# thunguyenphuoc/RenderNet

Hardware: AMD Instinct MI355X
Metric: rendered frames/sec, 64^3 voxel->512x512 Phong, batch 24 (higher is better)
Workload: dtype f32 (multiply stages: bf16x3-split operands, fp32 accumulate); 1 GPU; Phong shader forward (resampler + RenderNet 1-ch head), 5 shipped binvox fixtures cycled, 64^3 -> 128^3 -> 512x512, seeded random weights (237.3M params); batch_per_gpu=24, global_batch=24

## Files before the change

rendernet_amd/csrc/conv3d_wino_bf3.hip:

```cpp
#include "wino_xform.h"
#include <stdlib.h>
#include <type_traits>

typedef _Float16 f16x2 __attribute__((ext_vector_type(2)));

namespace {
constexpr int C3 = 32;
constexpr int C3PW = 34, C3PH = 4;
constexpr int C3NPIX = C3PW * C3PH;
constexpr int C3NPIECE = 17;
constexpr int C3STAGE = 18 * 1024;
constexpr int C3NSTG = 3;
constexpr int C3XCH = 4 * 2 * 2 * 2 * 1024;
constexpr int C3TAB = 256;
constexpr unsigned C3OOB = 0x80000000u;
}

struct C3Args {
    const float* x; const char* u; const float* bias; const float* alpha; const float* res; float* y; float* z;
    unsigned x_bytes;
    int B, H, W, D;
    int bh, bw;
    int nitems;
    int nseg, seglen;
    int act;
    const unsigned* amax_x; const unsigned* amax_u;
    unsigned* amax_y;
};

struct C3B3 : rnf::FmtB3 {};
struct C3H2 : rnf::FmtH2 {};
constexpr float C3_BOUND_X = 4.f, C3_BOUND_U = 2.25f;

__host__ __device__ inline float c3_h2_scale(float amax, float bound)
{
    const float t = amax * bound * (1.0f / 32768.0f);
    if (!(t > 0.f)) return 1.f;
    int e;
    const float m = frexpf(t, &e);
    return ldexpf(1.f, m == 0.5f ? e - 1 : e);
}

__global__ __launch_bounds__(256)
void conv3d_wino_pack_bf3_kernel(const float* __restrict__ w_tf, unsigned short* __restrict__ us, int transposed)
{
    const int idx = blockIdx.x * blockDim.x + threadIdx.x;
    if (idx >= 16 * 3 * C3 * C3) return;
    const int n = idx % C3, c = (idx / C3) % C3, dz = (idx / (C3 * C3)) % 3, xi = idx / (C3 * C3 * 3);
    const int i = xi >> 2, j = xi & 3;
    const double G[4][3] = {{1.0, 0.0, 0.0}, {0.5, 0.5, 0.5}, {0.5, -0.5, 0.5}, {0.0, 0.0, 1.0}};
    double acc = 0.0;
    for (int p = 0; p < 3; ++p)
        for (int q = 0; q < 3; ++q) {
            const float w = transposed ? w_tf[((((size_t)(2 - p) * 3 + (2 - q)) * 3 + (2 - dz)) * C3 + n) * C3 + c]
                                       : w_tf[((((size_t)p * 3 + q) * 3 + dz) * C3 + c) * C3 + n];
            acc = __builtin_fma(G[i][p] * G[j][q], (double)w, acc);
        }
    const float u = (float)acc;
    const __bf16 h0 = (__bf16)u;
    const float r1 = u - (float)h0;
    const __bf16 h1 = (__bf16)r1;
    const float r2 = r1 - (float)h1;
    const __bf16 h2 = (__bf16)r2;
    const __bf16 h[3] = {h0, h1, h2};
    const int lane = (n & 15) + 16 * (c >> 3), nt = n >> 4, e = c & 7;
    for (int p = 0; p < 3; ++p)
        us[((((((size_t)i * 4 + j) * 3 + dz) * 3 + p) * 2 + nt) * 64 + lane) * 8 + e] = __builtin_bit_cast(unsigned short, h[p]);
}

__global__ __launch_bounds__(256)
void conv3d_wino_pack_h2_kernel(const float* __restrict__ w_tf, unsigned short* __restrict__ us, const unsigned* __restrict__ amax, int transposed)
{
    const int idx = blockIdx.x * blockDim.x + threadIdx.x;
    if (idx >= 16 * 3 * C3 * C3) return;
    const float inv = 1.f / c3_h2_scale(__builtin_bit_cast(float, *amax), C3_BOUND_U);
    const int n = idx % C3, c = (idx / C3) % C3, dz = (idx / (C3 * C3)) % 3, xi = idx / (C3 * C3 * 3);
    const int i = xi >> 2, j = xi & 3;
    const double G[4][3] = {{1.0, 0.0, 0.0}, {0.5, 0.5, 0.5}, {0.5, -0.5, 0.5}, {0.0, 0.0, 1.0}};
    double acc = 0.0;
    for (int p = 0; p < 3; ++p)
        for (int q = 0; q < 3; ++q) {
            const float w = transposed ? w_tf[((((size_t)(2 - p) * 3 + (2 - q)) * 3 + (2 - dz)) * C3 + n) * C3 + c]
                                       : w_tf[((((size_t)p * 3 + q) * 3 + dz) * C3 + c) * C3 + n];
            acc = __builtin_fma(G[i][p] * G[j][q], (double)w, acc);
        }
    const float u = (float)acc * inv;
    const _Float16 h0 = (_Float16)u;
    const _Float16 h1 = (_Float16)(u - (float)h0);
    const _Float16 h[2] = {h0, h1};
    const int lane = (n & 15) + 16 * (c >> 3), nt = n >> 4, e = c & 7;
    for (int p = 0; p < 2; ++p)
        us[((((((size_t)i * 4 + j) * 3 + dz) * 2 + p) * 2 + nt) * 64 + lane) * 8 + e] = __builtin_bit_cast(unsigned short, h[p]);
}

__device__ __forceinline__ void c3_split8(const f32x4 lo, const f32x4 hi, bf16x8 (&p)[3])
{
#pragma unroll
    for (int e = 0; e < 8; e += 2) {
        f32x2 v = e < 4 ? f32x2{lo[e], lo[e + 1]} : f32x2{hi[e - 4], hi[e - 3]};
        const bf16x2 h0 = __builtin_convertvector(v, bf16x2);
        v -= __builtin_convertvector(h0, f32x2);
        const bf16x2 h1 = __builtin_convertvector(v, bf16x2);
        v -= __builtin_convertvector(h1, f32x2);
        const bf16x2 h2 = __builtin_convertvector(v, bf16x2);
        p[0][e] = h0[0]; p[0][e + 1] = h0[1];
        p[1][e] = h1[0]; p[1][e + 1] = h1[1];
        p[2][e] = h2[0]; p[2][e + 1] = h2[1];
    }
}

__device__ __forceinline__ void c3_split8(const f32x4 lo, const f32x4 hi, float inv, f16x8 (&p)[2])
{
#pragma unroll
    for (int e = 0; e < 8; e += 2) {
        f32x2 v = (e < 4 ? f32x2{lo[e], lo[e + 1]} : f32x2{hi[e - 4], hi[e - 3]}) * inv;
        const f16x2 h0 = __builtin_convertvector(v, f16x2);
        v -= __builtin_convertvector(h0, f32x2);
        const f16x2 h1 = __builtin_convertvector(v, f16x2);
        p[0][e] = h0[0]; p[0][e + 1] = h0[1];
        p[1][e] = h1[0]; p[1][e + 1] = h1[1];
    }
}
__device__ __forceinline__ void c3_split8(const f32x4 lo, const f32x4 hi, float, bf16x8 (&p)[3]) { c3_split8(lo, hi, p); }

__device__ __forceinline__ void c3_mfma(f32x4& c, const bf16x8& u, const bf16x8& p)
{
    asm("s_nop 1\n\tv_mfma_f32_16x16x32_bf16 %0, %1, %2, %0" : "+v"(c) : "a"(u), "v"(p));
}
__device__ __forceinline__ void c3_mfma_start(f32x4& c, const bf16x8& u, const bf16x8& p)
{
    asm("s_nop 1\n\tv_mfma_f32_16x16x32_bf16 %0, %1, %2, 0" : "=v"(c) : "v"(u), "v"(p));
}
__device__ __forceinline__ void c3_mfma(f32x4& c, const f16x8& u, const f16x8& p)
{
    asm("s_nop 1\n\tv_mfma_f32_16x16x32_f16 %0, %1, %2, %0" : "+v"(c) : "a"(u), "v"(p));
}
__device__ __forceinline__ void c3_mfma_start(f32x4& c, const f16x8& u, const f16x8& p)
{
    asm("s_nop 1\n\tv_mfma_f32_16x16x32_f16 %0, %1, %2, 0" : "=v"(c) : "a"(u), "v"(p));
}

__device__ __forceinline__ int c3_slot_swap(int px) { return ((px >> 4) | (px >> 5)) & 1; }

#define C3_WAIT_BARRIER(N) asm volatile("s_waitcnt vmcnt(" #N ") lgkmcnt(0)\n\ts_barrier" ::: "memory")

template <class F, bool AMAX>
__global__ __launch_bounds__(512, 1)
void conv3d_wino_bf3_kernel(const C3Args a)
{
    typedef typename F::frag frag;
    constexpr int NP = F::NP;
#if defined(__HIP_DEVICE_COMPILE__)
    extern __shared__ __attribute__((aligned(16))) char smem[];
    typedef __attribute__((address_space(3))) void lds_void;
    typedef unsigned u32x4 __attribute__((ext_vector_type(4)));
    const int tid = threadIdx.x;
    const int lane = tid & 63, wave = __builtin_amdgcn_readfirstlane(tid >> 6);
    const int r = wave >> 1, c = wave & 1;
    const int tx = lane & 15, kq = lane >> 4;
    const __amdgpu_buffer_rsrc_t xrsrc = __builtin_amdgcn_make_buffer_rsrc(const_cast<float*>(a.x), 0, a.x_bytes, 0x00020000);
    const __amdgpu_buffer_rsrc_t yrsrc = __builtin_amdgcn_make_buffer_rsrc(a.y, 0, a.x_bytes, 0x00020000);
    const __amdgpu_buffer_rsrc_t zrsrc = __builtin_amdgcn_make_buffer_rsrc(a.z ? a.z : a.y, 0, a.x_bytes, 0x00020000);
    const __amdgpu_buffer_rsrc_t rrsrc = __builtin_amdgcn_make_buffer_rsrc(const_cast<float*>(a.res ? a.res : a.x), 0, a.x_bytes, 0x00020000);

    frag U[2][3][NP][2];
    {
        const frag* up = reinterpret_cast<const frag*>(a.u) + (size_t)(r * 4 + 2 * c) * (3 * NP * 2 * 64) + lane;
#pragma unroll
        for (int jj = 0; jj < 2; ++jj)
#pragma unroll
            for (int dz = 0; dz < 3; ++dz)
#pragma unroll
                for (int p = 0; p < NP; ++p)
#pragma unroll
                    for (int nt = 0; nt < 2; ++nt) U[jj][dz][p][nt] = up[(((jj * 3 + dz) * NP + p) * 2 + nt) * 64];
    }
    float inv_x = 1.f, out_scale = 1.f;
    if constexpr (F::ID == 1) {
        const float sx = c3_h2_scale(__builtin_bit_cast(float, *a.amax_x), C3_BOUND_X);
        inv_x = 1.f / sx;
        out_scale = sx * c3_h2_scale(__builtin_bit_cast(float, *a.amax_u), C3_BOUND_U);
    }
    float ymax = 0.f;
    float* tab = reinterpret_cast<float*>(smem + C3NSTG * C3STAGE + 2 * C3XCH);
    if (tid < C3) {
        tab[tid] = a.bias ? a.bias[tid] : 0.f;
        tab[C3 + tid] = a.alpha ? a.alpha[tid] : 0.f;
    }
    const int rowA = (0x1210 >> (4 * r)) & 3, rowB = (0x3122 >> (4 * r)) & 3;
    const float sgn = r == 1 ? 1.f : -1.f;
    unsigned fo[3][2];
#pragma unroll
    for (int k = 0; k < 3; ++k)
#pragma unroll
        for (int h = 0; h < 2; ++h) {
            const int b = c + k;
            const int px = 2 * tx + b;
            fo[k][h] = (unsigned)((px ^ c3_slot_swap(px)) * 128) + ((((unsigned)(2 * kq + h)) ^ (unsigned)((px >> 1) & 7)) << 4);
        }
    const unsigned offA = (unsigned)(rowA * C3PW * 128), offB = (unsigned)(rowB * C3PW * 128);

    const int G = gridDim.x;
    const unsigned pix_bytes = (unsigned)a.D * (C3 * 4);
    const bool three = wave == 0;
    const int ent = wave >> 2, dy = (wave >> 1) & 1, dx = wave & 1;
    const int nch = ent * 16 + 4 * kq;
    __syncthreads();

    f32x4 acc[3][2][2];
    const int perm = (int)(blockIdx.x & 7) * (G >> 3) + (int)(blockIdx.x >> 3);
    for (int id = perm; id < a.nitems; id += G) {
        const int bx = id % a.bw, by = (id / a.bw) % a.bh, bi = (id / (a.bw * a.bh)) % a.B, seg = id / (a.bw * a.bh * a.B);
        const int o0 = seg * a.seglen, o1 = o0 + a.seglen < a.D ? o0 + a.seglen : a.D;
        if (o0 >= o1) continue;
        const int ds = o0 > 0 ? o0 - 1 : 0, dl = o1 < a.D ? o1 : a.D - 1;
        const int y0 = by * 2 - 1, x0 = bx * 32 - 1;
        const unsigned base = (unsigned)((bi * a.H + y0) * a.W + x0) * pix_bytes;
        unsigned roff[3];
#pragma unroll
        for (int i = 0; i < 3; ++i) {
            const int q = (wave + 8 * i) * 8 + (lane >> 3);
            const int py = (q * 241) >> 13, pxs = q - py * C3PW;
            const int px = pxs ^ c3_slot_swap(pxs);
            const bool ok = q < C3NPIX && (unsigned)(y0 + py) < (unsigned)a.H && (unsigned)(x0 + px) < (unsigned)a.W;
            roff[i] = ok ? base + (unsigned)(py * a.W + px) * pix_bytes + (unsigned)((((lane & 7) ^ ((px >> 1) & 7))) << 4) : C3OOB;
        }
        const int oy = by * 2 + dy, ox = bx * 32 + 2 * tx + dx;
        const unsigned ooff = (oy < a.H && ox < a.W) ? (unsigned)((bi * a.H + oy) * a.W + ox) * pix_bytes + (unsigned)(nch * 4) : C3OOB;

        auto issue = [&](int d, int stage) {
            char* sb = smem + stage * C3STAGE;
#pragma unroll
            for (int i = 0; i < 3; ++i) {
                if (i == 2 && !three) break;
                __builtin_amdgcn_raw_ptr_buffer_load_lds(xrsrc, (lds_void*)(sb + (wave + 8 * i) * 1024), 16,
                                                         roff[i] + (unsigned)(d * (C3 * 4)), 0, 0, 0);
            }
        };
        auto wait_newest = [&](bool issued) {
            if (!issued) C3_WAIT_BARRIER(0);
            else if (three) C3_WAIT_BARRIER(3);
            else C3_WAIT_BARRIER(2);
        };
        issue(ds, 0);
        if (ds + 1 <= dl) issue(ds + 1, 1);
#pragma unroll
        for (int jj = 0; jj < 2; ++jj)
#pragma unroll
            for (int nt = 0; nt < 2; ++nt) acc[0][jj][nt] = f32x4{0.f, 0.f, 0.f, 0.f};
        wait_newest(ds + 1 <= dl);

        auto step = [&](auto sc, int d) {
            constexpr int S = decltype(sc)::value;
            constexpr int SP = (S + 2) % 3, SN = (S + 1) % 3;
            const bool fl = d > o0;
            const bool arith = d <= dl;
            f32x4 rv = {0.f, 0.f, 0.f, 0.f};
            if (fl && a.res) rv = __builtin_bit_cast(f32x4, __builtin_amdgcn_raw_buffer_load_b128(rrsrc, ooff, (d - 1) * (C3 * 4), 0));
            asm volatile("" ::: "memory");
            const bool issued = d + 2 <= dl;
            if (issued) issue(d + 2, SP);
            if (arith) {
                const char* sb = smem + S * C3STAGE;
                f32x4 v[2][2];
#pragma unroll
                for (int h = 0; h < 2; ++h) {
                    f32x4 t[3];
#pragma unroll
                    for (int k = 0; k < 3; ++k) {
                        const f32x4 dA = *reinterpret_cast<const f32x4*>(sb + fo[k][h] + offA);
                        const f32x4 dB = *reinterpret_cast<const f32x4*>(sb + fo[k][h] + offB);
                        t[k] = dA + sgn * dB;
                    }
                    if (c == 0) { v[0][h] = t[0] - t[2]; v[1][h] = t[1] + t[2]; }
                    else        { v[0][h] = t[1] - t[0]; v[1][h] = t[0] - t[2]; }
                }
#pragma unroll
                for (int jj = 0; jj < 2; ++jj) {
                    frag p[NP];
                    c3_split8(v[jj][0], v[jj][1], inv_x, p);
#pragma unroll
                    for (int k = 0; k < F::NPROD; ++k)
#pragma unroll
                        for (int nt = 0; nt < 2; ++nt) {
                            c3_mfma(acc[SP][jj][nt], U[jj][2][F::PU[k]][nt], p[F::PV[k]]);
                            c3_mfma(acc[S][jj][nt], U[jj][1][F::PU[k]][nt], p[F::PV[k]]);
                            if (k == 0) c3_mfma_start(acc[SN][jj][nt], U[jj][0][F::PU[k]][nt], p[F::PV[k]]);
                            else c3_mfma(acc[SN][jj][nt], U[jj][0][F::PU[k]][nt], p[F::PV[k]]);
                        }
                }
            }
            char* xch = smem + C3NSTG * C3STAGE + (d & 1) * C3XCH;
            if (fl) {
                asm volatile("s_nop 15\n\ts_nop 15" : "+v"(acc[SP][0][0]), "+v"(acc[SP][0][1]), "+v"(acc[SP][1][0]), "+v"(acc[SP][1][1]) :: "memory");
#pragma unroll
                for (int nt = 0; nt < 2; ++nt) {
                    const f32x4 m0 = acc[SP][0][nt], m1 = acc[SP][1][nt], s = m0 + m1;
                    const f32x4 p0 = c == 0 ? s : m0, p1 = c == 0 ? m1 : -s;
                    *reinterpret_cast<f32x4*>(xch + ((((r * 2 + 0) * 2 + c) * 2 + nt) * 64 + lane) * 16) = p0;
                    *reinterpret_cast<f32x4*>(xch + ((((r * 2 + 1) * 2 + c) * 2 + nt) * 64 + lane) * 16) = p1;
                }
            }
            wait_newest(issued);
            if (fl) {
                f32x4 ci[3];
#pragma unroll
                for (int k = 0; k < 3; ++k)
                    ci[k] = *reinterpret_cast<const f32x4*>(xch + (((((dy + k) * 2 + dx) * 2 + 0) * 2 + ent) * 64 + lane) * 16)
                          + *reinterpret_cast<const f32x4*>(xch + (((((dy + k) * 2 + dx) * 2 + 1) * 2 + ent) * 64 + lane) * 16);
                f32x4 o = (dy == 0 ? (ci[0] + ci[1]) + ci[2] : (ci[0] - ci[1]) - ci[2]);
                if constexpr (F::ID == 1) o *= out_scale;
                o += *reinterpret_cast<const f32x4*>(tab + nch);
                const unsigned so = ooff + (unsigned)((d - 1) * (C3 * 4));
                if (a.z) __builtin_amdgcn_raw_buffer_store_b128(__builtin_bit_cast(u32x4, o), zrsrc, so, 0, 0);
                if (a.act & RN_ACT_PRELU) {
                    const f32x4 av = *reinterpret_cast<const f32x4*>(tab + C3 + nch);
#pragma unroll
                    for (int e = 0; e < 4; ++e) o[e] = fmaxf(o[e], 0.f) + av[e] * fminf(o[e], 0.f);
                }
                if (a.act & RN_ACT_ELU) {
#pragma unroll
                    for (int e = 0; e < 4; ++e) o[e] = o[e] > 0.f ? o[e] : expf(o[e]) - 1.f;
                }
                if (a.res) o += rv;
                if (a.act & RN_ACT_SIGMOID) {
#pragma unroll
                    for (int e = 0; e < 4; ++e) o[e] = 1.f / (1.f + __expf(-o[e]));
                }
                __builtin_amdgcn_raw_buffer_store_b128(__builtin_bit_cast(u32x4, o), yrsrc, so, 0, 0);
                if (AMAX && ooff != C3OOB) ymax = fmaxf(fmaxf(ymax, fmaxf(fabsf(o[0]), fabsf(o[1]))), fmaxf(fabsf(o[2]), fabsf(o[3])));
            }
        };
        for (int d = ds; d <= o1; d += 3) {
            step(std::integral_constant<int, 0>{}, d);
            if (d + 1 <= o1) step(std::integral_constant<int, 1>{}, d + 1);
            if (d + 2 <= o1) step(std::integral_constant<int, 2>{}, d + 2);
        }
    }
    if (AMAX) {
#pragma unroll
        for (int o = 32; o > 0; o >>= 1) ymax = fmaxf(ymax, __shfl_xor(ymax, o));
        if (lane == 0) atomicMax(a.amax_y, __builtin_bit_cast(unsigned, ymax));
    }
#endif
}

bool rn_conv3d_wino_bf3_supported(int Cin, int Cout)
{
    return Cin == C3 && Cout == C3;
}

size_t rn_conv3d_wino_bf3_packed_bytes() { return (size_t)16 * 3 * C3 * C3 * 3 * 2; }
size_t rn_conv3d_wino_split_packed_bytes(int fmt) { return fmt == 1 ? (size_t)16 * 3 * C3 * C3 * 2 * 2 + 256 : rn_conv3d_wino_bf3_packed_bytes(); }

int rn_launch_conv3d_wino_pack_bf3(const float* w_tf, void* us, int transposed, hipStream_t st)
{
    return rn_launch_conv3d_wino_split_pack(0, w_tf, us, transposed, st);
}

int rn_launch_conv3d_wino_split_pack(int fmt, const float* w_tf, void* us, int transposed, hipStream_t st)
{
    if (fmt == 1) {
        unsigned* amax = reinterpret_cast<unsigned*>(static_cast<char*>(us) + (size_t)16 * 3 * C3 * C3 * 2 * 2);
        const int rc = rn_launch_absmax(w_tf, (size_t)27 * C3 * C3, amax, st);
        if (rc != RN_OK) return rc;
        hipLaunchKernelGGL(conv3d_wino_pack_h2_kernel, dim3((16 * 3 * C3 * C3 + 255) / 256), dim3(256), 0, st, w_tf,
                           static_cast<unsigned short*>(us), amax, transposed);
        return rn_check_launch("conv3d_wino_pack_h2");
    }
    hipLaunchKernelGGL(conv3d_wino_pack_bf3_kernel, dim3((16 * 3 * C3 * C3 + 255) / 256), dim3(256), 0, st, w_tf,
                       static_cast<unsigned short*>(us), transposed);
    return rn_check_launch("conv3d_wino_pack_bf3");
}

int rn_launch_conv3d_wino_bf3(const float* x, const void* us, const float* bias, const float* alpha, const float* residual,
                              float* y, float* preact, int B, int H, int W, int D, int act, hipStream_t st)
{
    return rn_launch_conv3d_wino_split(0, x, us, bias, alpha, residual, y, preact, B, H, W, D, act, nullptr, nullptr, nullptr, st);
}

static int c3_depth_segments(long long rows, int D)
{
    static const int forced = getenv("RN_C3_DEPTH_SEGMENTS") ? atoi(getenv("RN_C3_DEPTH_SEGMENTS")) : 0;
    if (forced >= 1) return forced < D ? forced : D;
    int best = 1;
    long long best_cost = 0;
    for (int n = 1; n <= 8 && n <= D; n *= 2) {
        const int len = (D + n - 1) / n;
        const long long rounds = (rows * n + 255) / 256;
        const long long cost = rounds * (len + (n > 1 ? 2 : 1) + 1);
        if (n == 1 || cost < best_cost) { best = n; best_cost = cost; }
    }
    return best;
}

int rn_launch_conv3d_wino_split(int fmt, const float* x, const void* us, const float* bias, const float* alpha, const float* residual,
                                float* y, float* preact, int B, int H, int W, int D, int act, const unsigned* amax_x, unsigned* scratch_amax,
                                unsigned* amax_y, hipStream_t st)
{
    if (B < 1 || H < 1 || W < 1 || D < 1) return rn_set_error(RN_E_INVALID, "conv3d_wino_bf3: bad sizes");
    if ((act & RN_ACT_PRELU) && !alpha) return rn_set_error(RN_E_INVALID, "conv3d_wino_bf3: PReLU needs alpha");
    if (fmt < 0 || fmt > 1) return rn_set_error(RN_E_INVALID, "conv3d_wino_bf3: operand format %d", fmt);
    const size_t per_image = (size_t)H * W * D * C3 * 4;
    if (per_image >= 0x7fffff00ULL) return rn_set_error(RN_E_UNSUPPORTED, "conv3d_wino_bf3: one image exceeds the 2 GiB buffer window");
    const int chunk = (int)(0x7fffff00ULL / per_image);
    const size_t lds = (size_t)C3NSTG * C3STAGE + 2 * C3XCH + C3TAB;
    void (*kern)(const C3Args) = fmt == 1 ? (amax_y ? conv3d_wino_bf3_kernel<C3H2, true> : conv3d_wino_bf3_kernel<C3H2, false>)
                                          : (amax_y ? conv3d_wino_bf3_kernel<C3B3, true> : conv3d_wino_bf3_kernel<C3B3, false>);
    { const int rc_ = rn_ensure_dynamic_lds(reinterpret_cast<const void*>(kern), lds); if (rc_ != RN_OK) return rc_; }
    if (fmt == 1 && !amax_x) {
        if (!scratch_amax) return rn_set_error(RN_E_INVALID, "conv3d_wino_bf3: format H2 needs max|x| or a word to gather it in");
        const int rc = rn_launch_absmax(x, (size_t)B * H * W * D * C3, scratch_amax, st);
        if (rc != RN_OK) return rc;
        amax_x = scratch_amax;
    }
    if (amax_y) { const int rc = rn_launch_word(amax_y, nullptr, st); if (rc != RN_OK) return rc; }
    for (int b0 = 0; b0 < B; b0 += chunk) {
        const int nb = B - b0 < chunk ? B - b0 : chunk;
        const size_t off = (size_t)b0 * H * W * D * C3;
        C3Args a;
        a.x = x + off; a.u = static_cast<const char*>(us); a.bias = bias; a.alpha = alpha; a.res = residual ? residual + off : nullptr;
        a.y = y + off; a.z = preact ? preact + off : nullptr;
        a.x_bytes = (unsigned)(nb * per_image);
        a.B = nb; a.H = H; a.W = W; a.D = D;
        a.bh = (H + 1) / 2; a.bw = (W + 31) / 32;
        const long long rows = (long long)nb * a.bh * a.bw;
        a.nseg = c3_depth_segments(rows, D);
        a.seglen = (D + a.nseg - 1) / a.nseg;
        const long long nitems = rows * a.nseg;
        if (nitems > 0x7fffffffLL) return rn_set_error(RN_E_UNSUPPORTED, "conv3d_wino_bf3: too many items (%lld rows x %d depth segments)", rows, a.nseg);
        a.nitems = (int)nitems; a.act = act;
        a.amax_x = amax_x; a.amax_y = amax_y;
        a.amax_u = fmt == 1 ? reinterpret_cast<const unsigned*>(static_cast<const char*>(us) + (size_t)16 * 3 * C3 * C3 * 2 * 2) : nullptr;
        const unsigned grid = nitems < 256 ? (unsigned)((nitems + 7) / 8 * 8) : 256u;
        hipLaunchKernelGGL(kern, dim3(grid), dim3(512), lds, st, a);
        const int rc = rn_check_launch("conv3d_wino_bf3");
        if (rc != RN_OK) return rc;
    }
    return RN_OK;
}
```

Measured before the change: 331.4 frames/s.

## Pipeline depth-loop across work items so prefetch and epilogue span item boundaries

Turns the per-item depth loop of the Winograd 3D conv into one continuous software pipeline. Separate fetch and arithmetic cursors let the next item's first slices be prefetched while the current item finishes, and the last output slice's epilogue overlaps with the next item's first compute. This removes the pipeline fill and drain stall at every item boundary. The depth-segment cost model drops its per-item fill penalty and nseg is recomputed from seglen, so segment choice may change. The price is more complex state tracking, extra register pressure, and kernarg reloads on each item switch.

New measurement: 331.0 frames/s. Within noise of the previous version (-0.1%).

```diff
diff --git a/rendernet_amd/csrc/conv3d_wino_bf3.hip b/rendernet_amd/csrc/conv3d_wino_bf3.hip
--- a/rendernet_amd/csrc/conv3d_wino_bf3.hip
+++ b/rendernet_amd/csrc/conv3d_wino_bf3.hip
@@ -209,132 +209,184 @@
 
     f32x4 acc[3][2][2];
     const int perm = (int)(blockIdx.x & 7) * (G >> 3) + (int)(blockIdx.x >> 3);
-    for (int id = perm; id < a.nitems; id += G) {
-        const int bx = id % a.bw, by = (id / a.bw) % a.bh, bi = (id / (a.bw * a.bh)) % a.B, seg = id / (a.bw * a.bh * a.B);
-        const int o0 = seg * a.seglen, o1 = o0 + a.seglen < a.D ? o0 + a.seglen : a.D;
-        if (o0 >= o1) continue;
-        const int ds = o0 > 0 ? o0 - 1 : 0, dl = o1 < a.D ? o1 : a.D - 1;
+    int fid = perm, fd = 0, fdl = -1;
+    int fvalid = 0;
+    unsigned roff[3];
+    auto args = [&]() {
+        typedef const __attribute__((address_space(4))) C3Args* kptr;
+        kptr k = (kptr)__builtin_amdgcn_kernarg_segment_ptr();
+        asm volatile("" : "+s"(k));
+        return k;
+    };
+    auto open_fetch = [&]() {
+        const auto* k = args();
+        const int bw = k->bw, bh = k->bh, nb = k->B, sl = k->seglen, nd = k->D, ah = k->H, aw = k->W;
+        const int bx = fid % bw, by = (fid / bw) % bh, bi = (fid / (bw * bh)) % nb, seg = fid / (bw * bh * nb);
+        const int o0 = seg * sl, o1 = o0 + sl < nd ? o0 + sl : nd;
+        fd = o0 > 0 ? o0 - 1 : 0; fdl = o1 < nd ? o1 : nd - 1;
         const int y0 = by * 2 - 1, x0 = bx * 32 - 1;
-        const unsigned base = (unsigned)((bi * a.H + y0) * a.W + x0) * pix_bytes;
-        unsigned roff[3];
+        const unsigned base = (unsigned)((bi * ah + y0) * aw + x0) * pix_bytes;
+        int ln = lane;
+        asm volatile("" : "+v"(ln));
 #pragma unroll
         for (int i = 0; i < 3; ++i) {
-            const int q = (wave + 8 * i) * 8 + (lane >> 3);
+            const int q = (wave + 8 * i) * 8 + (ln >> 3);
             const int py = (q * 241) >> 13, pxs = q - py * C3PW;
             const int px = pxs ^ c3_slot_swap(pxs);
-            const bool ok = q < C3NPIX && (unsigned)(y0 + py) < (unsigned)a.H && (unsigned)(x0 + px) < (unsigned)a.W;
-            roff[i] = ok ? base + (unsigned)(py * a.W + px) * pix_bytes + (unsigned)((((lane & 7) ^ ((px >> 1) & 7))) << 4) : C3OOB;
-        }
-        const int oy = by * 2 + dy, ox = bx * 32 + 2 * tx + dx;
-        const unsigned ooff = (oy < a.H && ox < a.W) ? (unsigned)((bi * a.H + oy) * a.W + ox) * pix_bytes + (unsigned)(nch * 4) : C3OOB;
-
-        auto issue = [&](int d, int stage) {
-            char* sb = smem + stage * C3STAGE;
-#pragma unroll
-            for (int i = 0; i < 3; ++i) {
-                if (i == 2 && !three) break;
-                __builtin_amdgcn_raw_ptr_buffer_load_lds(xrsrc, (lds_void*)(sb + (wave + 8 * i) * 1024), 16,
-                                                         roff[i] + (unsigned)(d * (C3 * 4)), 0, 0, 0);
+            const bool ok = q < C3NPIX && (unsigned)(y0 + py) < (unsigned)ah && (unsigned)(x0 + px) < (unsigned)aw;
+            roff[i] = ok ? base + (unsigned)(py * aw + px) * pix_bytes + (unsigned)((((ln & 7) ^ ((px >> 1) & 7))) << 4) : C3OOB;
+        }
+    };
+    auto fetch = [&](int stage) {
+        char* sb = smem + stage * C3STAGE;
+#pragma unroll
+        for (int i = 0; i < 3; ++i) {
+            if (i == 2 && !three) break;
+            __builtin_amdgcn_raw_ptr_buffer_load_lds(xrsrc, (lds_void*)(sb + (wave + 8 * i) * 1024), 16,
+                                                     roff[i] + (unsigned)(fd * (C3 * 4)), 0, 0, 0);
+        }
+        if (++fd > fdl) {
+            fid += G;
+            fvalid = fid < args()->nitems;
+            if (fvalid) open_fetch();
+        }
+    };
+    auto wait_newest = [&](bool issued) {
+        if (!issued) C3_WAIT_BARRIER(0);
+        else if (three) C3_WAIT_BARRIER(3);
+        else C3_WAIT_BARRIER(2);
+    };
+    int aid = perm, d = 0, dl = -1, o0 = 0, o1 = 0;
+    int arith = 0, first = 0;
+    unsigned ooff = C3OOB;
+    auto open_arith = [&]() {
+        const auto* k = args();
+        const int bw = k->bw, bh = k->bh, nb = k->B, sl = k->seglen, nd = k->D, ah = k->H, aw = k->W;
+        const int bx = aid % bw, by = (aid / bw) % bh, bi = (aid / (bw * bh)) % nb, seg = aid / (bw * bh * nb);
+        o0 = seg * sl; o1 = o0 + sl < nd ? o0 + sl : nd;
+        d = o0 > 0 ? o0 - 1 : 0; dl = o1 < nd ? o1 : nd - 1;
+        first = 1;
+        int ln = lane;
+        asm volatile("" : "+v"(ln));
+        const int oy = by * 2 + dy, ox = bx * 32 + 2 * (ln & 15) + dx;
+        ooff = (oy < ah && ox < aw) ? (unsigned)((bi * ah + oy) * aw + ox) * pix_bytes + (unsigned)((ent * 16 + 4 * (ln >> 4)) * 4) : C3OOB;
+    };
+    int fl = 0;
+    int fsl = 0, xsel = 0;
+    unsigned foff = C3OOB;
+
+    auto step = [&](auto sc) {
+        constexpr int S = decltype(sc)::value;
+        constexpr int SP = (S + 2) % 3, SN = (S + 1) % 3;
+        f32x4 rv = {0.f, 0.f, 0.f, 0.f};
+        if (fl && a.res) rv = __builtin_bit_cast(f32x4, __builtin_amdgcn_raw_buffer_load_b128(rrsrc, foff, fsl * (C3 * 4), 0));
+        asm volatile("" ::: "memory");
+        const bool issued = fvalid;
+        if (issued) fetch(SP);
+        char* xch = smem + C3NSTG * C3STAGE + xsel * C3XCH;
+        auto put = [&]() {
+            asm volatile("s_nop 15\n\ts_nop 15" : "+v"(acc[SP][0][0]), "+v"(acc[SP][0][1]), "+v"(acc[SP][1][0]), "+v"(acc[SP][1][1]) :: "memory");
+#pragma unroll
+            for (int nt = 0; nt < 2; ++nt) {
+                const f32x4 m0 = acc[SP][0][nt], m1 = acc[SP][1][nt], s = m0 + m1;
+                const f32x4 p0 = c == 0 ? s : m0, p1 = c == 0 ? m1 : -s;
+                *reinterpret_cast<f32x4*>(xch + ((((r * 2 + 0) * 2 + c) * 2 + nt) * 64 + lane) * 16) = p0;
+                *reinterpret_cast<f32x4*>(xch + ((((r * 2 + 1) * 2 + c) * 2 + nt) * 64 + lane) * 16) = p1;
             }
         };
-        auto wait_newest = [&](bool issued) {
-            if (!issued) C3_WAIT_BARRIER(0);
-            else if (three) C3_WAIT_BARRIER(3);
-            else C3_WAIT_BARRIER(2);
-        };
-        issue(ds, 0);
-        if (ds + 1 <= dl) issue(ds + 1, 1);
-#pragma unroll
-        for (int jj = 0; jj < 2; ++jj)
-#pragma unroll
-            for (int nt = 0; nt < 2; ++nt) acc[0][jj][nt] = f32x4{0.f, 0.f, 0.f, 0.f};
-        wait_newest(ds + 1 <= dl);
-
-        auto step = [&](auto sc, int d) {
-            constexpr int S = decltype(sc)::value;
-            constexpr int SP = (S + 2) % 3, SN = (S + 1) % 3;
-            const bool fl = d > o0;
-            const bool arith = d <= dl;
-            f32x4 rv = {0.f, 0.f, 0.f, 0.f};
-            if (fl && a.res) rv = __builtin_bit_cast(f32x4, __builtin_amdgcn_raw_buffer_load_b128(rrsrc, ooff, (d - 1) * (C3 * 4), 0));
-            asm volatile("" ::: "memory");
-            const bool issued = d + 2 <= dl;
-            if (issued) issue(d + 2, SP);
-            if (arith) {
-                const char* sb = smem + S * C3STAGE;
-                f32x4 v[2][2];
-#pragma unroll
-                for (int h = 0; h < 2; ++h) {
-                    f32x4 t[3];
-#pragma unroll
-                    for (int k = 0; k < 3; ++k) {
-                        const f32x4 dA = *reinterpret_cast<const f32x4*>(sb + fo[k][h] + offA);
-                        const f32x4 dB = *reinterpret_cast<const f32x4*>(sb + fo[k][h] + offB);
-                        t[k] = dA + sgn * dB;
+        if (fl && first) put();
+        if (arith) {
+            if (d == 0) {
+#pragma unroll
+                for (int jj = 0; jj < 2; ++jj)
+#pragma unroll
+                    for (int nt = 0; nt < 2; ++nt) acc[S][jj][nt] = f32x4{0.f, 0.f, 0.f, 0.f};
+            }
+            const char* sb = smem + S * C3STAGE;
+            f32x4 v[2][2];
+#pragma unroll
+            for (int h = 0; h < 2; ++h) {
+                f32x4 t[3];
+#pragma unroll
+                for (int k = 0; k < 3; ++k) {
+                    const f32x4 dA = *reinterpret_cast<const f32x4*>(sb + fo[k][h] + offA);
+                    const f32x4 dB = *reinterpret_cast<const f32x4*>(sb + fo[k][h] + offB);
+                    t[k] = dA + sgn * dB;
+                }
+                if (c == 0) { v[0][h] = t[0] - t[2]; v[1][h] = t[1] + t[2]; }
+                else        { v[0][h] = t[1] - t[0]; v[1][h] = t[0] - t[2]; }
+            }
+#pragma unroll
+            for (int jj = 0; jj < 2; ++jj) {
+                frag p[NP];
+                c3_split8(v[jj][0], v[jj][1], inv_x, p);
+#pragma unroll
+                for (int k = 0; k < F::NPROD; ++k)
+#pragma unroll
+                    for (int nt = 0; nt < 2; ++nt) {
+                        c3_mfma(acc[SP][jj][nt], U[jj][2][F::PU[k]][nt], p[F::PV[k]]);
+                        c3_mfma(acc[S][jj][nt], U[jj][1][F::PU[k]][nt], p[F::PV[k]]);
+                        if (k == 0) c3_mfma_start(acc[SN][jj][nt], U[jj][0][F::PU[k]][nt], p[F::PV[k]]);
+                        else c3_mfma(acc[SN][jj][nt], U[jj][0][F::PU[k]][nt], p[F::PV[k]]);
                     }
-                    if (c == 0) { v[0][h] = t[0] - t[2]; v[1][h] = t[1] + t[2]; }
-                    else        { v[0][h] = t[1] - t[0]; v[1][h] = t[0] - t[2]; }
-                }
-#pragma unroll
-                for (int jj = 0; jj < 2; ++jj) {
-                    frag p[NP];
-                    c3_split8(v[jj][0], v[jj][1], inv_x, p);
-#pragma unroll
-                    for (int k = 0; k < F::NPROD; ++k)
-#pragma unroll
-                        for (int nt = 0; nt < 2; ++nt) {
-                            c3_mfma(acc[SP][jj][nt], U[jj][2][F::PU[k]][nt], p[F::PV[k]]);
-                            c3_mfma(acc[S][jj][nt], U[jj][1][F::PU[k]][nt], p[F::PV[k]]);
-                            if (k == 0) c3_mfma_start(acc[SN][jj][nt], U[jj][0][F::PU[k]][nt], p[F::PV[k]]);
-                            else c3_mfma(acc[SN][jj][nt], U[jj][0][F::PU[k]][nt], p[F::PV[k]]);
-                        }
-                }
-            }
-            char* xch = smem + C3NSTG * C3STAGE + (d & 1) * C3XCH;
-            if (fl) {
-                asm volatile("s_nop 15\n\ts_nop 15" : "+v"(acc[SP][0][0]), "+v"(acc[SP][0][1]), "+v"(acc[SP][1][0]), "+v"(acc[SP][1][1]) :: "memory");
-#pragma unroll
-                for (int nt = 0; nt < 2; ++nt) {
-                    const f32x4 m0 = acc[SP][0][nt], m1 = acc[SP][1][nt], s = m0 + m1;
-                    const f32x4 p0 = c == 0 ? s : m0, p1 = c == 0 ? m1 : -s;
-                    *reinterpret_cast<f32x4*>(xch + ((((r * 2 + 0) * 2 + c) * 2 + nt) * 64 + lane) * 16) = p0;
-                    *reinterpret_cast<f32x4*>(xch + ((((r * 2 + 1) * 2 + c) * 2 + nt) * 64 + lane) * 16) = p1;
-                }
-            }
-            wait_newest(issued);
-            if (fl) {
-                f32x4 ci[3];
-#pragma unroll
-                for (int k = 0; k < 3; ++k)
-                    ci[k] = *reinterpret_cast<const f32x4*>(xch + (((((dy + k) * 2 + dx) * 2 + 0) * 2 + ent) * 64 + lane) * 16)
-                          + *reinterpret_cast<const f32x4*>(xch + (((((dy + k) * 2 + dx) * 2 + 1) * 2 + ent) * 64 + lane) * 16);
-                f32x4 o = (dy == 0 ? (ci[0] + ci[1]) + ci[2] : (ci[0] - ci[1]) - ci[2]);
-                if constexpr (F::ID == 1) o *= out_scale;
-                o += *reinterpret_cast<const f32x4*>(tab + nch);
-                const unsigned so = ooff + (unsigned)((d - 1) * (C3 * 4));
-                if (a.z) __builtin_amdgcn_raw_buffer_store_b128(__builtin_bit_cast(u32x4, o), zrsrc, so, 0, 0);
-                if (a.act & RN_ACT_PRELU) {
-                    const f32x4 av = *reinterpret_cast<const f32x4*>(tab + C3 + nch);
-#pragma unroll
-                    for (int e = 0; e < 4; ++e) o[e] = fmaxf(o[e], 0.f) + av[e] * fminf(o[e], 0.f);
-                }
-                if (a.act & RN_ACT_ELU) {
-#pragma unroll
-                    for (int e = 0; e < 4; ++e) o[e] = o[e] > 0.f ? o[e] : expf(o[e]) - 1.f;
-                }
-                if (a.res) o += rv;
-                if (a.act & RN_ACT_SIGMOID) {
-#pragma unroll
-                    for (int e = 0; e < 4; ++e) o[e] = 1.f / (1.f + __expf(-o[e]));
-                }
-                __builtin_amdgcn_raw_buffer_store_b128(__builtin_bit_cast(u32x4, o), yrsrc, so, 0, 0);
-                if (AMAX && ooff != C3OOB) ymax = fmaxf(fmaxf(ymax, fmaxf(fabsf(o[0]), fabsf(o[1]))), fmaxf(fabsf(o[2]), fabsf(o[3])));
-            }
-        };
-        for (int d = ds; d <= o1; d += 3) {
-            step(std::integral_constant<int, 0>{}, d);
-            if (d + 1 <= o1) step(std::integral_constant<int, 1>{}, d + 1);
-            if (d + 2 <= o1) step(std::integral_constant<int, 2>{}, d + 2);
+            }
+        }
+        if (fl && !first) put();
+        wait_newest(issued);
+        if (fl) {
+            f32x4 ci[3];
+#pragma unroll
+            for (int k = 0; k < 3; ++k)
+                ci[k] = *reinterpret_cast<const f32x4*>(xch + (((((dy + k) * 2 + dx) * 2 + 0) * 2 + ent) * 64 + lane) * 16)
+                      + *reinterpret_cast<const f32x4*>(xch + (((((dy + k) * 2 + dx) * 2 + 1) * 2 + ent) * 64 + lane) * 16);
+            f32x4 o = (dy == 0 ? (ci[0] + ci[1]) + ci[2] : (ci[0] - ci[1]) - ci[2]);
+            if constexpr (F::ID == 1) o *= out_scale;
+            o += *reinterpret_cast<const f32x4*>(tab + nch);
+            const unsigned so = foff + (unsigned)(fsl * (C3 * 4));
+            if (a.z) __builtin_amdgcn_raw_buffer_store_b128(__builtin_bit_cast(u32x4, o), zrsrc, so, 0, 0);
+            if (a.act & RN_ACT_PRELU) {
+                const f32x4 av = *reinterpret_cast<const f32x4*>(tab + C3 + nch);
+#pragma unroll
+                for (int e = 0; e < 4; ++e) o[e] = fmaxf(o[e], 0.f) + av[e] * fminf(o[e], 0.f);
+            }
+            if (a.act & RN_ACT_ELU) {
+#pragma unroll
+                for (int e = 0; e < 4; ++e) o[e] = o[e] > 0.f ? o[e] : expf(o[e]) - 1.f;
+            }
+            if (a.res) o += rv;
+            if (a.act & RN_ACT_SIGMOID) {
+#pragma unroll
+                for (int e = 0; e < 4; ++e) o[e] = 1.f / (1.f + __expf(-o[e]));
+            }
+            __builtin_amdgcn_raw_buffer_store_b128(__builtin_bit_cast(u32x4, o), yrsrc, so, 0, 0);
+            if (AMAX && foff != C3OOB) ymax = fmaxf(fmaxf(ymax, fmaxf(fabsf(o[0]), fabsf(o[1]))), fmaxf(fabsf(o[2]), fabsf(o[3])));
+        }
+        xsel ^= 1;
+        fl = arith && d >= o0 && d < o1;
+        fsl = d; foff = ooff;
+        if (arith) {
+            first = 0;
+            if (++d > dl) {
+                aid += G;
+                arith = aid < args()->nitems;
+                if (arith) open_arith();
+            }
+        }
+    };
+    if (perm < a.nitems) {
+        fvalid = 1; open_fetch();
+        arith = 1; open_arith();
+        fetch(0);
+        const bool two = fvalid;
+        if (two) fetch(1);
+        wait_newest(two);
+        for (;;) {
+            step(std::integral_constant<int, 0>{});
+            if (!(arith || fl)) break;
+            step(std::integral_constant<int, 1>{});
+            if (!(arith || fl)) break;
+            step(std::integral_constant<int, 2>{});
+            if (!(arith || fl)) break;
         }
     }
     if (AMAX) {
@@ -388,7 +440,7 @@
     for (int n = 1; n <= 8 && n <= D; n *= 2) {
         const int len = (D + n - 1) / n;
         const long long rounds = (rows * n + 255) / 256;
-        const long long cost = rounds * (len + (n > 1 ? 2 : 1) + 1);
+        const long long cost = rounds * (len + (n > 1 ? 2 : 0)) + 2;
         if (n == 1 || cost < best_cost) { best = n; best_cost = cost; }
     }
     return best;
@@ -427,6 +479,7 @@
         const long long rows = (long long)nb * a.bh * a.bw;
         a.nseg = c3_depth_segments(rows, D);
         a.seglen = (D + a.nseg - 1) / a.nseg;
+        a.nseg = (D + a.seglen - 1) / a.seglen;
         const long long nitems = rows * a.nseg;
         if (nitems > 0x7fffffffLL) return rn_set_error(RN_E_UNSUPPORTED, "conv3d_wino_bf3: too many items (%lld rows x %d depth segments)", rows, a.nseg);
         a.nitems = (int)nitems; a.act = act;
```
